# amzn/MXFusion

Measured on AMD Instinct MI355X. Metric: ELBO-steps/sec + RBF Gram GB/s, SVGP N=65k D=8 M=1024, 1->8 MI355X, higher is better.
Workload: dtype f32; 1 GPU; SVGPRegression RBF-ARD N=65536 Q=8 M=1024, 32 MC samples (latent-input model), StochasticVariationalInference step = draw + ELBO + reverse mode + grad all-reduce + Adam; samples_per_gpu=32, parallelism=mc-samples sharded x1, 1 RCCL all-reduce of the flat gradient/step, core_precision=float64 (M x M factorisations), streaming float32

## Files before the change

### mxfusion_amd/csrc/gemm_bt.hip

```cpp
#include "common.h"
#include "internal.h"
#include "split_device.h"

namespace {

typedef short s16x4 __attribute__((ext_vector_type(4)));

struct BtArgs {
    const unsigned short* A; const unsigned short* Bt; float* C;
    int64_t M, N, K16;
    int64_t pA, pB, btR;
    float alpha;
    int c_blk;
    int64_t ldc;
    int64_t tm, tn, nwg;
    const float* ad0;
    const unsigned* maxbits;
    const unsigned* maxbits2;
    unsigned* maxout;
    unsigned* sync; int sync_n;
    int sync_every;
    const unsigned short* uw; const unsigned* uwmax; float* uout; float uscale;
};

__device__ __forceinline__ void bt_dma16(const void* sbase, unsigned voff, unsigned lds) {
    asm volatile("s_mov_b32 m0, %2\n\ts_nop 0\n\tglobal_load_lds_dwordx4 %0, %1" ::"v"(voff), "s"(sbase), "s"(lds) : "memory", "m0");
}

__device__ __forceinline__ float bt_dot8(u32x4 a, u32x4 b, float acc) {
    const f16x8 av = __builtin_bit_cast(f16x8, a), bv = __builtin_bit_cast(f16x8, b);
    acc = __builtin_amdgcn_fdot2(f16x2{av[0], av[1]}, f16x2{bv[0], bv[1]}, acc, false);
    acc = __builtin_amdgcn_fdot2(f16x2{av[2], av[3]}, f16x2{bv[2], bv[3]}, acc, false);
    acc = __builtin_amdgcn_fdot2(f16x2{av[4], av[5]}, f16x2{bv[4], bv[5]}, acc, false);
    acc = __builtin_amdgcn_fdot2(f16x2{av[6], av[7]}, f16x2{bv[6], bv[7]}, acc, false);
    return acc;
}

constexpr int BT_KMAX16 = 128;

template <bool WU>
__global__ __launch_bounds__(512, 2) void gemm_f16x2_bt_kernel(BtArgs g) {
    constexpr int NU = 512;
    __shared__ u32x4 sA[4][2][NU];
    __shared__ u32x4 sB[4][2][NU];
    __shared__ u32x4 sW[WU ? 2 * BT_KMAX16 * 2 : 1];
    __shared__ float sU[WU ? 512 : 1];
    const int tid = threadIdx.x, lane = tid & 63, wave = tid >> 6, wq = wave & 3, wh = wave >> 2;
    const int li = lane & 31, lk = lane >> 5;
    int patience = 2;
    float cmax = 0.f;
    if constexpr (WU) {
        if (g.uout) {
            const int nunits = (int)(g.K16 * 2);
            for (int i = tid; i < 2 * nunits; i += 512) {
                const int p = i / nunits, u = i % nunits;
                sW[p * (BT_KMAX16 * 2) + u] = *reinterpret_cast<const u32x4*>(g.uw + (int64_t)p * g.K16 * 16 + u * 8);
            }
        }
        __syncthreads();
    }
    float alpha = g.alpha;
    if (g.ad0) alpha *= g.ad0[0];
    if (g.maxbits) alpha /= scale_from_maxbits(g.maxbits[0]);
    if (g.maxbits2) alpha /= scale_from_maxbits(g.maxbits2[0]);

    const int drow = tid >> 1, dkh = (tid & 1) ^ ((drow >> 3) & 1);
    const int bc = tid >> 3, bs = tid & 7;
    const int b_nb = 4 * (bc >> 4) + 2 * ((bc >> 3) & 1) + (bc & 1);
    const int b_kl = 8 * ((bc >> 1) & 1) + 4 * ((bc >> 2) & 1) + (bs >> 1);
    const unsigned voff_b = (unsigned)((((int64_t)b_nb * g.btR + b_kl) * 16 + 8 * (bs & 1)) * 2);
    const unsigned voff_a = (unsigned)((drow * 16 + dkh * 8) * 2);
    const int ua0_ = lds_unit(128 * wh + li, lk);
#define ua_(x) (ua0_ + 64 * (x))
    const unsigned ldsA = __builtin_amdgcn_readfirstlane((unsigned)(size_t)(__attribute__((address_space(3))) void*)&sA[0][0][wave * 64]);
    const unsigned ldsB = __builtin_amdgcn_readfirstlane((unsigned)(size_t)(__attribute__((address_space(3))) void*)&sB[0][0][wave * 64]);
    const unsigned toff_blk = (unsigned)((((int64_t)(4 * wq) * g.M + 128 * wh + li) * 16 + 4 * lk) * 4);
    const int rb_h = (wq * 2048 + (lane >> 4) * 128 + ((lane & 15) >> 2) * 32 + (lane & 3) * 8) / 2;

    const int nk = (int)g.K16;
    const unsigned nwg = (unsigned)g.nwg, tmu = (unsigned)g.tm;
    const int nit = (int)((nwg - blockIdx.x + gridDim.x - 1) / gridDim.x);
    const int nsteps = nit * nk;
    const unsigned q8 = nwg / 8, r8 = nwg % 8;
    auto item_of = [&](int i) -> unsigned { return xcd_run_item(blockIdx.x + (unsigned)i * gridDim.x, q8, r8); };
    int q_it = 0, q_kb = 0;
    unsigned q_slot = 0;
    const unsigned short* qa = nullptr;
    const unsigned short* qb = nullptr;
    auto q_enter = [&]() {
        const unsigned wid = item_of(q_it);
        const unsigned tn_ = wid / tmu, tm_ = wid - tn_ * tmu;
        qa = g.A + (int64_t)tm_ * 256 * 16;
        qb = g.Bt + ((int64_t)tn_ * 16) * g.btR * 16;
    };
    auto q_issue = [&]() {
        bt_dma16(qa + (int64_t)q_kb * g.M * 16, voff_a, ldsA + q_slot * 16384);
        bt_dma16(qa + g.pA + (int64_t)q_kb * g.M * 16, voff_a, ldsA + q_slot * 16384 + 8192);
        bt_dma16(qb + (int64_t)q_kb * 256, voff_b, ldsB + q_slot * 16384);
        bt_dma16(qb + g.pB + (int64_t)q_kb * 256, voff_b, ldsB + q_slot * 16384 + 8192);
        q_slot = (q_slot + 1) & 3;
        if (++q_kb == nk) { q_kb = 0; ++q_it; if (q_it < nit) q_enter(); }
    };
#define BT_WAIT(NSTR) do { asm volatile("s_waitcnt vmcnt(" NSTR ")" ::: "memory"); __builtin_amdgcn_s_barrier(); asm volatile("" ::: "memory"); } while (0)
#define HF(v) __builtin_bit_cast(f16x8, v)
#define BT_TR(ptr) __builtin_bit_cast(u32x2, __builtin_amdgcn_ds_read_tr16_b64_v4i16((__attribute__((address_space(3))) s16x4*)(ptr)))
    f32x16 c[4][2];
    float ua0 = 0.f, ua1 = 0.f;
    int c_kb = 0, c_it = 0;
    int64_t m0 = 0, n0 = 0;
    unsigned c_slot = 0;
    bool uitem = false;
    u32x4 fb0[2][2], fa0[2];
    u32x4 dga[6];
#define BT_READ_B(FB, SLOTV)                                                                                                        \
    do {                                                                                                                            \
        _Pragma("unroll") for (int p = 0; p < 2; ++p) {                                                                             \
            const unsigned short* sb_ = reinterpret_cast<const unsigned short*>(&sB[SLOTV][p][0]) + rb_h;                           \
            _Pragma("unroll") for (int y = 0; y < 2; ++y) {                                                                         \
                const u32x2 v0_ = BT_TR(sb_ + (2 * y) * 256), v1_ = BT_TR(sb_ + (2 * y + 1) * 256);                                 \
                FB[y][p] = u32x4{v0_[0], v0_[1], v1_[0], v1_[1]};                                                                   \
            }                                                                                                                       \
        }                                                                                                                           \
    } while (0)
#define BT_READ_A0(FA, SLOTV) do { FA[0] = sA[SLOTV][0][ua_(0)]; FA[1] = sA[SLOTV][1][ua_(0)]; } while (0)
#define BT_MM(x, AH, AL, FB)                                                                                                        \
    do {                                                                                                                            \
        _Pragma("unroll") for (int y = 0; y < 2; ++y) {                                                                             \
            c[x][y] = __builtin_amdgcn_mfma_f32_32x32x16_f16(HF(FB[y][0]), HF(AL), c[x][y], 0, 0, 0);                   \
            c[x][y] = __builtin_amdgcn_mfma_f32_32x32x16_f16(HF(FB[y][1]), HF(AH), c[x][y], 0, 0, 0);                   \
            c[x][y] = __builtin_amdgcn_mfma_f32_32x32x16_f16(HF(FB[y][0]), HF(AH), c[x][y], 0, 0, 0);                   \
        }                                                                                                                           \
    } while (0)
#define BT_STEP(FB, FA)                                                                                                   \
    do {                                                                                                                            \
        if (c_kb == 0) {                                                                        \
            const unsigned wid = item_of(c_it);                                                                                     \
            const unsigned tile_n = wid / tmu, tile_m = wid - tile_n * tmu;                                                         \
            m0 = (int64_t)tile_m * 256; n0 = (int64_t)tile_n * 256;                                                                 \
            uitem = WU && g.uout != nullptr && ((tile_n + (tile_n >> 3) + (tile_n >> 6)) % tmu) == tile_m;                          \
            if (g.sync && (c_it % g.sync_every) == 0) wg_rendezvous(g.sync + wid / g.sync_n, (unsigned)g.sync_n, patience);         \
            _Pragma("unroll") for (int x = 0; x < 4; ++x)                                                                           \
                _Pragma("unroll") for (int y = 0; y < 2; ++y)                                                                       \
                    _Pragma("unroll") for (int r = 0; r < 16; ++r) c[x][y][r] = 0.f;                                                \
            ua0 = 0.f; ua1 = 0.f;                                                                                                   \
        }                                                                                                                           \
        const bool more = s_ + 3 < nsteps;                                                                                          \
        if (more) q_issue();                                                      \
        asm volatile("" ::: "memory");                                             \
        const unsigned nslot = (c_slot + 1) & 3;                                                                                    \
        BT_READ_B(FB, c_slot);                                                                                                      \
        BT_READ_A0(FA, c_slot);                                                                                                     \
        if constexpr (WU) {                                                                                                         \
            if (uitem && (((int)c_kb & 1) == wh)) {                              \
                const u32x4 wh_ = sW[2 * (int)c_kb + lk], wl_ = sW[BT_KMAX16 * 2 + 2 * (int)c_kb + lk];                             \
                ua0 = bt_dot8(FB[0][1], wh_, ua0); ua0 = bt_dot8(FB[0][0], wl_, ua0); ua0 = bt_dot8(FB[0][0], wh_, ua0);            \
                ua1 = bt_dot8(FB[1][1], wh_, ua1); ua1 = bt_dot8(FB[1][0], wl_, ua1); ua1 = bt_dot8(FB[1][0], wh_, ua1);            \
            }                                                                                                                       \
        }                                                                                                                           \
         \
        dga[0] = sA[c_slot][0][ua_(1)]; dga[1] = sA[c_slot][1][ua_(1)]; dga[2] = sA[c_slot][0][ua_(2)]; dga[3] = sA[c_slot][1][ua_(2)];      \
        u32x4 a1h = dga[0], a1l = dga[1];                                                                                           \
        u32x4 a2h = dga[2], a2l = dga[3];                                                                                           \
        BT_MM(0, FA[0], FA[1], FB);                                                                                                 \
        __builtin_amdgcn_sched_barrier(0);               \
        dga[4] = sA[c_slot][0][ua_(3)]; dga[5] = sA[c_slot][1][ua_(3)];                                                             \
        u32x4 a3h = dga[4], a3l = dga[5];                                                                                           \
        BT_MM(1, a1h, a1l, FB);                                                                                                     \
        __builtin_amdgcn_sched_barrier(0);                                                                                          \
        BT_MM(2, a2h, a2l, FB);                                                                                                     \
        __builtin_amdgcn_sched_barrier(0);                                                                                          \
        BT_MM(3, a3h, a3l, FB);                                                                                                     \
        __builtin_amdgcn_sched_barrier(0);                                                                                          \
        if (more) BT_WAIT("8"); else if (s_ + 2 < nsteps) BT_WAIT("4"); else BT_WAIT("0");                        \
        c_slot = nslot;                                                                                                             \
        if (++c_kb == nk) { c_kb = 0; ++c_it; finish_item(); }                                                                      \
        ++s_;                                                                                                                       \
    } while (0)
    auto finish_item = [&]() {
        if constexpr (WU) {
            if (uitem) {
                ua0 += __shfl_xor(ua0, 32, 64);
                ua1 += __shfl_xor(ua1, 32, 64);
                if (lane < 32) { sU[256 * wh + 64 * wq + li] = ua0; sU[256 * wh + 64 * wq + 32 + li] = ua1; }
                __syncthreads();
                if (tid < 256) {
                    float sc = g.uscale * (g.ad0 ? g.ad0[0] : 1.f) / scale_from_maxbits(g.uwmax[0]);
                    if (g.maxbits2) sc /= scale_from_maxbits(g.maxbits2[0]);
                    g.uout[n0 + tid] = (sU[tid] + sU[256 + tid]) * sc;
                }
            }
        }
        if (g.c_blk) {
            char* const cb = reinterpret_cast<char*>(g.C) + ((n0 >> 4) * g.M + m0) * 64;
#pragma unroll
            for (int x = 0; x < 4; ++x)
#pragma unroll
                for (int y = 0; y < 2; ++y)
#pragma unroll
                    for (int q = 0; q < 4; ++q) {
                        char* const sb = cb + ((int64_t)(2 * y + (q >> 1)) * g.M + 32 * x) * 64 + 32 * (q & 1);
                        const f32x4 v = {alpha * c[x][y][4 * q], alpha * c[x][y][4 * q + 1], alpha * c[x][y][4 * q + 2], alpha * c[x][y][4 * q + 3]};
                        *reinterpret_cast<f32x4*>(sb + toff_blk) = v;
                        if (g.maxout) cmax = fmaxf(fmaxf(cmax, fmaxf(fabsf(v[0]), fabsf(v[1]))), fmaxf(fabsf(v[2]), fabsf(v[3])));
                    }
        } else {
#pragma unroll
            for (int x = 0; x < 4; ++x) {
                const int64_t row = m0 + 128 * wh + 32 * x + li;
#pragma unroll
                for (int y = 0; y < 2; ++y)
#pragma unroll
                    for (int q = 0; q < 4; ++q) {
                        const int64_t col = n0 + 64 * wq + 32 * y + 8 * q + 4 * lk;
                        float* p = g.C + row * g.ldc + col;
                        const f32x4 v = {alpha * c[x][y][4 * q], alpha * c[x][y][4 * q + 1], alpha * c[x][y][4 * q + 2], alpha * c[x][y][4 * q + 3]};
                        *reinterpret_cast<f32x4*>(p) = v;
                        if (g.maxout) cmax = fmaxf(fmaxf(cmax, fmaxf(fabsf(v[0]), fabsf(v[1]))), fmaxf(fabsf(v[2]), fabsf(v[3])));
                    }
            }
        }
    };
    if (nsteps > 0) {
        q_enter();
        q_issue();
        q_issue();
        q_issue();
        BT_WAIT("8");
    }
    int s_ = 0;
    while (s_ < nsteps) BT_STEP(fb0, fa0);
#undef ua_
#undef BT_STEP
#undef BT_MM
#undef BT_READ_A0
#undef BT_READ_B
#undef BT_TR
#undef HF
#undef BT_WAIT
    if (g.maxout) {
#pragma unroll
        for (int o = 32; o > 0; o >>= 1) cmax = fmaxf(cmax, __shfl_xor(cmax, o, 64));
        if (lane == 0 && __builtin_bit_cast(unsigned, cmax) > *(volatile unsigned*)g.maxout) atomicMax(g.maxout, __builtin_bit_cast(unsigned, cmax));
    }
}

__global__ __launch_bounds__(256) void bt_wsplit_kernel(int64_t K, int64_t Kp, const float* __restrict__ w, unsigned short* __restrict__ planes,
                                                        unsigned* __restrict__ maxword) {
    __shared__ unsigned wm[4];
    unsigned m = 0;
    for (int64_t i = threadIdx.x; i < K; i += 256) { const unsigned b = __builtin_bit_cast(unsigned, w[i]) & 0x7fffffffu; m = b > m ? b : m; }
    for (int o = 32; o > 0; o >>= 1) { const unsigned t = (unsigned)__shfl_xor((int)m, o); m = t > m ? t : m; }
    if ((threadIdx.x & 63) == 0) wm[threadIdx.x >> 6] = m;
    __syncthreads();
    for (int i = 0; i < 4; ++i) m = wm[i] > m ? wm[i] : m;
    if (threadIdx.x == 0) maxword[0] = m;
    const float sc = scale_from_maxbits(m);
    for (int64_t i = threadIdx.x; i < Kp; i += 256) {
        const float x = i < K ? w[i] * sc : 0.f;
        const _Float16 fh = (_Float16)x;
        const _Float16 fl = (_Float16)(x - (float)fh);
        planes[i] = __builtin_bit_cast(unsigned short, fh);
        planes[Kp + i] = __builtin_bit_cast(unsigned short, fl);
    }
}

}

bool mxf_gemm_bt_ok(int64_t M, int64_t N, int64_t K) { return M > 0 && N > 0 && K >= 48 && (M % 256) == 0 && (N % 256) == 0 && (K % 16) == 0; }

namespace {

struct BtPlan { BtArgs g; unsigned grid; unsigned ncounters; const float* w; unsigned short* wplanes; unsigned* wmax; };

int bt_plan(mxf_ctx* h, int64_t M, int64_t N, int64_t K, const MxfSplitScale& sc, const MxfPlanes& A, const MxfPlanes& Bt, int64_t btR,
            const MxfSplitOut& o, const MxfBtURow& u, const MxfSplitSched& sched, BtPlan& p) {
    if (o.planes || o.planes_t || o.avec || o.a_lower || o.lower_only || o.beta != 0.0 || sc.pow0 < 0 || sc.pow0 > 1)
        MXF_FAIL(h, -2, "mxf_gemm_bt: the output is C or blocked C of a full product with beta == 0, and ad0 enters once");
    if (o.blocked && M * 16 * 64 >= (1ll << 31)) MXF_FAIL(h, -3, "mxf_gemm_bt: too many rows for the blocked output");
    if (btR * 16 * 32 >= (1ll << 31)) MXF_FAIL(h, -3, "mxf_gemm_bt: the K-major operand has too many rows");
    if (!mxf_gemm_bt_ok(M, N, K) || btR < K) MXF_FAIL(h, -2, "mxf_gemm_bt: needs M %% 256 == 0, N %% 256 == 0, K %% 16 == 0, K >= 48");
    if (o.blocked && o.ldc != N) MXF_FAIL(h, -2, "mxf_gemm_bt: the blocked output layout needs ldc == N");
    if ((o.ldc % 4) != 0 || (((uintptr_t)o.C) % 16) != 0) MXF_FAIL(h, -2, "mxf_gemm_bt: C must be 16-byte aligned with ldc %% 4 == 0");
    if (u.U && (!u.w || !u.wscratch || K / 16 > BT_KMAX16)) MXF_FAIL(h, -2, "mxf_gemm_bt: the U row needs w, scratch and K <= %d", BT_KMAX16 * 16);
    BtArgs& g = p.g;
    memset(&g, 0, sizeof(g));
    g.A = A.p; g.pA = A.stride; g.maxbits = A.maxbits; g.Bt = Bt.p; g.pB = Bt.stride; g.maxbits2 = Bt.maxbits; g.btR = btR;
    g.M = M; g.N = N; g.K16 = K / 16; g.tm = M / 256; g.tn = N / 256; g.nwg = g.tm * g.tn;
    g.alpha = (float)sc.alpha; g.ad0 = sc.pow0 ? sc.ad0 : nullptr;
    g.C = o.C; g.ldc = o.ldc; g.c_blk = o.blocked; g.maxout = o.maxout;
    p.w = u.w; p.wplanes = nullptr; p.wmax = nullptr;
    if (u.U) {
        p.wplanes = (unsigned short*)u.wscratch; p.wmax = (unsigned*)(p.wplanes + 2 * K);
        g.uw = p.wplanes; g.uwmax = p.wmax; g.uout = u.U; g.uscale = (float)u.uscale;
    }
    int64_t grid = (int64_t)(256 - (sched.reserve_cus > 0 ? sched.reserve_cus : 0)) / 8 * 8;
    if (grid < 8) grid = 8;
    if (g.nwg <= grid) grid = g.nwg;
    p.grid = (unsigned)grid;
    static const int sync_env = (int)MXF_KNOB("MXF_BT_SYNC", 4);
    p.ncounters = 0;
    if (sync_env && strip_rendezvous_ok(g.tm, g.nwg, grid)) {
        p.ncounters = (unsigned)(g.nwg / g.tm);
        g.sync_n = (int)g.tm; g.sync_every = sync_env > 0 ? sync_env : 1;
    }
    return 0;
}

int bt_launch(mxf_ctx* h, hipStream_t st, BtPlan& p) {
    BtArgs& g = p.g;
    if (g.uout) hipLaunchKernelGGL(bt_wsplit_kernel, dim3(1), dim3(256), 0, st, g.K16 * 16, g.K16 * 16, p.w, p.wplanes, p.wmax);
    if (p.ncounters) g.sync = mxf_gsync(h, p.ncounters);
    if (g.uout) hipLaunchKernelGGL((gemm_f16x2_bt_kernel<true>), dim3(p.grid), dim3(512), 0, st, g);
    else hipLaunchKernelGGL((gemm_f16x2_bt_kernel<false>), dim3(p.grid), dim3(512), 0, st, g);
    MXF_LAUNCH_CHECK(h);
    return 0;
}

}

int mxf_gemm_bt_internal(mxf_ctx* h, hipStream_t st, int64_t M, int64_t N, int64_t K, MxfSplitScale scale, MxfPlanes A, MxfPlanes Bt, int64_t btR,
                         MxfSplitOut out, MxfBtURow u, MxfSplitSched sched) {
    BtPlan p;
    const int rc = bt_plan(h, M, N, K, scale, A, Bt, btR, out, u, sched, p);
    return rc ? rc : bt_launch(h, st, p);
}

extern "C" int mxf_gemm_f16x2_planes_kmajor(mxf_handle h, int64_t M, int64_t N, int64_t K, double alpha, const void* A_planes, const void* A_maxword,
                                            const void* Bt_planes, const void* Bt_maxword, void* C, int blocked, const void* w, void* U, void* stream) {
    if (!h) return -1;
    if (!A_planes || !Bt_planes || !A_maxword || !Bt_maxword || !C || ((w == nullptr) != (U == nullptr))) MXF_FAIL(h, -2, "mxf_gemm_f16x2_planes_kmajor: bad argument");
    if (!mxf_gemm_bt_ok(M, N, K)) MXF_FAIL(h, -3, "mxf_gemm_f16x2_planes_kmajor: needs M %% 256 == 0, N %% 256 == 0, K %% 16 == 0, K >= 48");
    void* ws = nullptr;
    if (U) {
        ws = mxf_ws(h, mxf_align((2 * (size_t)K + 8) * 2));
        if (!ws) MXF_FAIL(h, -4, "mxf_gemm_f16x2_planes_kmajor: cannot allocate scratch");
    }
    return mxf_gemm_bt_internal(h, (hipStream_t)stream, M, N, K, {.alpha = alpha},
                                {(const unsigned short*)A_planes, (int64_t)mxf_split_plane_elems(M, K), (const unsigned*)A_maxword},
                                {(const unsigned short*)Bt_planes, (int64_t)mxf_split_plane_elems(K, N), (const unsigned*)Bt_maxword}, K,
                                {.C = (float*)C, .ldc = N, .blocked = blocked ? 1 : 0}, {.w = (const float*)w, .U = (float*)U, .wscratch = ws});
}
```

Before: 43.54 ELBO-steps/sec.

## Switch BT GEMM to 16x16x32 MFMA with K-pair double-buffered stages

Replaces the 32x32x16 MFMA tiling with 16x16x32 MFMA. Each pipeline stage now loads two K16 blocks into a 2-slot double buffer instead of one block into a 4-slot ring. The A and B LDS layouts, the per-lane index math and the epilogue mappings are reworked to match, and the item loop is restructured around an odd-K tail that masks the upper half-lanes. The goal is fewer waits and barriers per unit of K work and better MFMA issue density. In exchange, register pressure rises (8x4 accumulators plus 8 fragments), prefetch depth drops, and the LDS reads for the next stage are interleaved with a mid-step barrier.

After: 44.92 ELBO-steps/sec, median of 6. +3.2%, better.

```diff
diff --git a/mxfusion_amd/csrc/gemm_bt.hip b/mxfusion_amd/csrc/gemm_bt.hip
--- a/mxfusion_amd/csrc/gemm_bt.hip
+++ b/mxfusion_amd/csrc/gemm_bt.hip
@@ -41,20 +41,20 @@
 template <bool WU>
 __global__ __launch_bounds__(512, 2) void gemm_f16x2_bt_kernel(BtArgs g) {
     constexpr int NU = 512;
-    __shared__ u32x4 sA[4][2][NU];
-    __shared__ u32x4 sB[4][2][NU];
+    __shared__ u32x4 sA[2][2][2][NU];
+    __shared__ u32x4 sB[2][2][2][NU];
     __shared__ u32x4 sW[WU ? 2 * BT_KMAX16 * 2 : 1];
     __shared__ float sU[WU ? 512 : 1];
     const int tid = threadIdx.x, lane = tid & 63, wave = tid >> 6, wq = wave & 3, wh = wave >> 2;
-    const int li = lane & 31, lk = lane >> 5;
+    const int lj = lane & 15, lg = lane >> 4;
     int patience = 2;
     float cmax = 0.f;
     if constexpr (WU) {
         if (g.uout) {
-            const int nunits = (int)(g.K16 * 2);
-            for (int i = tid; i < 2 * nunits; i += 512) {
-                const int p = i / nunits, u = i % nunits;
-                sW[p * (BT_KMAX16 * 2) + u] = *reinterpret_cast<const u32x4*>(g.uw + (int64_t)p * g.K16 * 16 + u * 8);
+            const int nunits = (int)(g.K16 * 2), npad = (nunits + 3) & ~3;
+            for (int i = tid; i < 2 * npad; i += 512) {
+                const int p = i / npad, u = i % npad;
+                sW[p * (BT_KMAX16 * 2) + u] = u < nunits ? *reinterpret_cast<const u32x4*>(g.uw + (int64_t)p * g.K16 * 16 + u * 8) : u32x4{0u, 0u, 0u, 0u};
             }
         }
         __syncthreads();
@@ -64,26 +64,24 @@
     if (g.maxbits) alpha /= scale_from_maxbits(g.maxbits[0]);
     if (g.maxbits2) alpha /= scale_from_maxbits(g.maxbits2[0]);
 
-    const int drow = tid >> 1, dkh = (tid & 1) ^ ((drow >> 3) & 1);
     const int bc = tid >> 3, bs = tid & 7;
-    const int b_nb = 4 * (bc >> 4) + 2 * ((bc >> 3) & 1) + (bc & 1);
-    const int b_kl = 8 * ((bc >> 1) & 1) + 4 * ((bc >> 2) & 1) + (bs >> 1);
+    const int b_nb = bc >> 2;
+    const int b_kl = 8 * (bc & 1) + 4 * ((bc >> 1) & 1) + (bs >> 1);
     const unsigned voff_b = (unsigned)((((int64_t)b_nb * g.btR + b_kl) * 16 + 8 * (bs & 1)) * 2);
-    const unsigned voff_a = (unsigned)((drow * 16 + dkh * 8) * 2);
-    const int ua0_ = lds_unit(128 * wh + li, lk);
-#define ua_(x) (ua0_ + 64 * (x))
-    const unsigned ldsA = __builtin_amdgcn_readfirstlane((unsigned)(size_t)(__attribute__((address_space(3))) void*)&sA[0][0][wave * 64]);
-    const unsigned ldsB = __builtin_amdgcn_readfirstlane((unsigned)(size_t)(__attribute__((address_space(3))) void*)&sB[0][0][wave * 64]);
-    const unsigned toff_blk = (unsigned)((((int64_t)(4 * wq) * g.M + 128 * wh + li) * 16 + 4 * lk) * 4);
-    const int rb_h = (wq * 2048 + (lane >> 4) * 128 + ((lane & 15) >> 2) * 32 + (lane & 3) * 8) / 2;
-
-    const int nk = (int)g.K16;
+    const unsigned voff_a = (unsigned)(tid * 16);
+    const int ua0_ = (128 * wh + lj) * 2 + (lg & 1) + (lg >> 1) * (2 * NU);
+    const unsigned ldsA = __builtin_amdgcn_readfirstlane((unsigned)(size_t)(__attribute__((address_space(3))) void*)&sA[0][0][0][wave * 64]);
+    const unsigned ldsB = __builtin_amdgcn_readfirstlane((unsigned)(size_t)(__attribute__((address_space(3))) void*)&sB[0][0][0][wave * 64]);
+    const unsigned toff_blk = (unsigned)((((int64_t)(4 * wq) * g.M + 128 * wh + lj) * 16 + 4 * lg) * 4);
+    const int rb_h = (wq * 2048 + (lg >> 1) * 16384 + (lg & 1) * 128 + (lj >> 2) * 32 + (lj & 3) * 8) / 2;
+
+    const int nk = (int)g.K16, np = (nk + 1) / 2;
     const unsigned nwg = (unsigned)g.nwg, tmu = (unsigned)g.tm;
     const int nit = (int)((nwg - blockIdx.x + gridDim.x - 1) / gridDim.x);
-    const int nsteps = nit * nk;
+    const int nsteps = nit * np;
     const unsigned q8 = nwg / 8, r8 = nwg % 8;
     auto item_of = [&](int i) -> unsigned { return xcd_run_item(blockIdx.x + (unsigned)i * gridDim.x, q8, r8); };
-    int q_it = 0, q_kb = 0;
+    int q_it = 0, q_p = 0;
     unsigned q_slot = 0;
     const unsigned short* qa = nullptr;
     const unsigned short* qb = nullptr;
@@ -94,94 +92,93 @@
         qb = g.Bt + ((int64_t)tn_ * 16) * g.btR * 16;
     };
     auto q_issue = [&]() {
-        bt_dma16(qa + (int64_t)q_kb * g.M * 16, voff_a, ldsA + q_slot * 16384);
-        bt_dma16(qa + g.pA + (int64_t)q_kb * g.M * 16, voff_a, ldsA + q_slot * 16384 + 8192);
-        bt_dma16(qb + (int64_t)q_kb * 256, voff_b, ldsB + q_slot * 16384);
-        bt_dma16(qb + g.pB + (int64_t)q_kb * 256, voff_b, ldsB + q_slot * 16384 + 8192);
-        q_slot = (q_slot + 1) & 3;
-        if (++q_kb == nk) { q_kb = 0; ++q_it; if (q_it < nit) q_enter(); }
+        const int kb0 = 2 * q_p, kb1 = kb0 + 1 < nk ? kb0 + 1 : kb0;
+        const unsigned la = ldsA + q_slot * 32768, lb = ldsB + q_slot * 32768;
+        bt_dma16(qa + (int64_t)kb0 * g.M * 16, voff_a, la);
+        bt_dma16(qa + g.pA + (int64_t)kb0 * g.M * 16, voff_a, la + 8192);
+        bt_dma16(qb + (int64_t)kb0 * 256, voff_b, lb);
+        bt_dma16(qb + g.pB + (int64_t)kb0 * 256, voff_b, lb + 8192);
+        bt_dma16(qa + (int64_t)kb1 * g.M * 16, voff_a, la + 16384);
+        bt_dma16(qa + g.pA + (int64_t)kb1 * g.M * 16, voff_a, la + 16384 + 8192);
+        bt_dma16(qb + (int64_t)kb1 * 256, voff_b, lb + 16384);
+        bt_dma16(qb + g.pB + (int64_t)kb1 * 256, voff_b, lb + 16384 + 8192);
+        q_slot ^= 1;
+        if (++q_p == np) { q_p = 0; ++q_it; if (q_it < nit) q_enter(); }
     };
 #define BT_WAIT(NSTR) do { asm volatile("s_waitcnt vmcnt(" NSTR ")" ::: "memory"); __builtin_amdgcn_s_barrier(); asm volatile("" ::: "memory"); } while (0)
 #define HF(v) __builtin_bit_cast(f16x8, v)
 #define BT_TR(ptr) __builtin_bit_cast(u32x2, __builtin_amdgcn_ds_read_tr16_b64_v4i16((__attribute__((address_space(3))) s16x4*)(ptr)))
-    f32x16 c[4][2];
-    float ua0 = 0.f, ua1 = 0.f;
-    int c_kb = 0, c_it = 0;
+    f32x4 c[8][4];
+    float ua[4] = {0.f, 0.f, 0.f, 0.f};
     int64_t m0 = 0, n0 = 0;
     unsigned c_slot = 0;
     bool uitem = false;
-    u32x4 fb0[2][2], fa0[2];
-    u32x4 dga[6];
-#define BT_READ_B(FB, SLOTV)                                                                                                        \
+    u32x4 fb[4][2];
+#define BT_A(x, p) sa_[(p) * NU + ua0_ + 32 * (x)]
+#define BT_MM(x, AH, AL)                                                                                                           \
     do {                                                                                                                            \
+        _Pragma("unroll") for (int t = 0; t < 4; ++t) {                                                                             \
+            c[x][t] = __builtin_amdgcn_mfma_f32_16x16x32_f16(HF(fb[t][0]), HF(AL), c[x][t], 0, 0, 0);                   \
+            c[x][t] = __builtin_amdgcn_mfma_f32_16x16x32_f16(HF(fb[t][1]), HF(AH), c[x][t], 0, 0, 0);                   \
+            c[x][t] = __builtin_amdgcn_mfma_f32_16x16x32_f16(HF(fb[t][0]), HF(AH), c[x][t], 0, 0, 0);                   \
+        }                                                                                                                           \
+        __builtin_amdgcn_sched_barrier(0);               \
+    } while (0)
+#define BT_STEP(TAIL)                                                                                                              \
+    do {                                                                                                                            \
+        const u32x4* const sa_ = &sA[c_slot][0][0][0];                                                                              \
         _Pragma("unroll") for (int p = 0; p < 2; ++p) {                                                                             \
-            const unsigned short* sb_ = reinterpret_cast<const unsigned short*>(&sB[SLOTV][p][0]) + rb_h;                           \
-            _Pragma("unroll") for (int y = 0; y < 2; ++y) {                                                                         \
-                const u32x2 v0_ = BT_TR(sb_ + (2 * y) * 256), v1_ = BT_TR(sb_ + (2 * y + 1) * 256);                                 \
-                FB[y][p] = u32x4{v0_[0], v0_[1], v1_[0], v1_[1]};                                                                   \
+            const unsigned short* sb_ = reinterpret_cast<const unsigned short*>(&sB[c_slot][0][p][0]) + rb_h;                       \
+            _Pragma("unroll") for (int t = 0; t < 4; ++t) {                                                                         \
+                const u32x2 v0_ = BT_TR(sb_ + t * 256), v1_ = BT_TR(sb_ + t * 256 + 128);                                           \
+                fb[t][p] = u32x4{v0_[0], v0_[1], v1_[0], v1_[1]};                                                                   \
+                if (TAIL) fb[t][p] &= kmask;            \
             }                                                                                                                       \
         }                                                                                                                           \
-    } while (0)
-#define BT_READ_A0(FA, SLOTV) do { FA[0] = sA[SLOTV][0][ua_(0)]; FA[1] = sA[SLOTV][1][ua_(0)]; } while (0)
-#define BT_MM(x, AH, AL, FB)                                                                                                        \
-    do {                                                                                                                            \
-        _Pragma("unroll") for (int y = 0; y < 2; ++y) {                                                                             \
-            c[x][y] = __builtin_amdgcn_mfma_f32_32x32x16_f16(HF(FB[y][0]), HF(AL), c[x][y], 0, 0, 0);                   \
-            c[x][y] = __builtin_amdgcn_mfma_f32_32x32x16_f16(HF(FB[y][1]), HF(AH), c[x][y], 0, 0, 0);                   \
-            c[x][y] = __builtin_amdgcn_mfma_f32_32x32x16_f16(HF(FB[y][0]), HF(AH), c[x][y], 0, 0, 0);                   \
-        }                                                                                                                           \
-    } while (0)
-#define BT_STEP(FB, FA)                                                                                                   \
-    do {                                                                                                                            \
-        if (c_kb == 0) {                                                                        \
-            const unsigned wid = item_of(c_it);                                                                                     \
-            const unsigned tile_n = wid / tmu, tile_m = wid - tile_n * tmu;                                                         \
-            m0 = (int64_t)tile_m * 256; n0 = (int64_t)tile_n * 256;                                                                 \
-            uitem = WU && g.uout != nullptr && ((tile_n + (tile_n >> 3) + (tile_n >> 6)) % tmu) == tile_m;                          \
-            if (g.sync && (c_it % g.sync_every) == 0) wg_rendezvous(g.sync + wid / g.sync_n, (unsigned)g.sync_n, patience);         \
-            _Pragma("unroll") for (int x = 0; x < 4; ++x)                                                                           \
-                _Pragma("unroll") for (int y = 0; y < 2; ++y)                                                                       \
-                    _Pragma("unroll") for (int r = 0; r < 16; ++r) c[x][y][r] = 0.f;                                                \
-            ua0 = 0.f; ua1 = 0.f;                                                                                                   \
-        }                                                                                                                           \
-        const bool more = s_ + 3 < nsteps;                                                                                          \
-        if (more) q_issue();                                                      \
-        asm volatile("" ::: "memory");                                             \
-        const unsigned nslot = (c_slot + 1) & 3;                                                                                    \
-        BT_READ_B(FB, c_slot);                                                                                                      \
-        BT_READ_A0(FA, c_slot);                                                                                                     \
+        u32x4 a0h = BT_A(0, 0), a0l = BT_A(0, 1), a1h = BT_A(1, 0), a1l = BT_A(1, 1);                                           \
         if constexpr (WU) {                                                                                                         \
-            if (uitem && (((int)c_kb & 1) == wh)) {                              \
-                const u32x4 wh_ = sW[2 * (int)c_kb + lk], wl_ = sW[BT_KMAX16 * 2 + 2 * (int)c_kb + lk];                             \
-                ua0 = bt_dot8(FB[0][1], wh_, ua0); ua0 = bt_dot8(FB[0][0], wl_, ua0); ua0 = bt_dot8(FB[0][0], wh_, ua0);            \
-                ua1 = bt_dot8(FB[1][1], wh_, ua1); ua1 = bt_dot8(FB[1][0], wl_, ua1); ua1 = bt_dot8(FB[1][0], wh_, ua1);            \
+            if (uitem && ((c_p & 1) == wh)) {                                 \
+                const u32x4 wh_ = sW[4 * c_p + lg], wl_ = sW[BT_KMAX16 * 2 + 4 * c_p + lg];                                         \
+                _Pragma("unroll") for (int t = 0; t < 4; ++t) {                                                                     \
+                    ua[t] = bt_dot8(fb[t][1], wh_, ua[t]); ua[t] = bt_dot8(fb[t][0], wl_, ua[t]); ua[t] = bt_dot8(fb[t][0], wh_, ua[t]); \
+                }                                                                                                                   \
             }                                                                                                                       \
         }                                                                                                                           \
-         \
-        dga[0] = sA[c_slot][0][ua_(1)]; dga[1] = sA[c_slot][1][ua_(1)]; dga[2] = sA[c_slot][0][ua_(2)]; dga[3] = sA[c_slot][1][ua_(2)];      \
-        u32x4 a1h = dga[0], a1l = dga[1];                                                                                           \
-        u32x4 a2h = dga[2], a2l = dga[3];                                                                                           \
-        BT_MM(0, FA[0], FA[1], FB);                                                                                                 \
-        __builtin_amdgcn_sched_barrier(0);               \
-        dga[4] = sA[c_slot][0][ua_(3)]; dga[5] = sA[c_slot][1][ua_(3)];                                                             \
-        u32x4 a3h = dga[4], a3l = dga[5];                                                                                           \
-        BT_MM(1, a1h, a1l, FB);                                                                                                     \
-        __builtin_amdgcn_sched_barrier(0);                                                                                          \
-        BT_MM(2, a2h, a2l, FB);                                                                                                     \
-        __builtin_amdgcn_sched_barrier(0);                                                                                          \
-        BT_MM(3, a3h, a3l, FB);                                                                                                     \
-        __builtin_amdgcn_sched_barrier(0);                                                                                          \
-        if (more) BT_WAIT("8"); else if (s_ + 2 < nsteps) BT_WAIT("4"); else BT_WAIT("0");                        \
-        c_slot = nslot;                                                                                                             \
-        if (++c_kb == nk) { c_kb = 0; ++c_it; finish_item(); }                                                                      \
-        ++s_;                                                                                                                       \
+                                                               \
+        u32x4 a2h = BT_A(2, 0), a2l = BT_A(2, 1);                                                                                 \
+        BT_MM(0, a0h, a0l);                                                                                                        \
+        u32x4 a3h = BT_A(3, 0), a3l = BT_A(3, 1);                                                                                 \
+        BT_MM(1, a1h, a1l);                                                                                                        \
+        u32x4 a4h = BT_A(4, 0), a4l = BT_A(4, 1);                                                                                 \
+        BT_MM(2, a2h, a2l);                                                                                                        \
+        u32x4 a5h = BT_A(5, 0), a5l = BT_A(5, 1);                                                                                 \
+        BT_MM(3, a3h, a3l);                                                                                                        \
+        u32x4 a6h = BT_A(6, 0), a6l = BT_A(6, 1);                                                                                 \
+        BT_MM(4, a4h, a4l);                                                                                                        \
+        u32x4 a7h = BT_A(7, 0), a7l = BT_A(7, 1);                                                                                 \
+        BT_MM(5, a5h, a5l);                                                                                                        \
+                     \
+        asm volatile("s_waitcnt lgkmcnt(0)" ::: "memory");                                                                          \
+        __builtin_amdgcn_s_barrier();                                                                                               \
+        asm volatile("" ::: "memory");                                                                                              \
+        const bool more = s_ + 2 < nsteps;                                                                                          \
+        if (more) q_issue();                                                                                                        \
+        asm volatile("" ::: "memory");                                                                                              \
+        BT_MM(6, a6h, a6l);                                                                                                        \
+        BT_MM(7, a7h, a7l);                                                                                                        \
+            \
+        if (more) BT_WAIT("8"); else BT_WAIT("0");                                                                                  \
+        c_slot ^= 1; ++c_p; ++s_;                                                                                                   \
     } while (0)
     auto finish_item = [&]() {
         if constexpr (WU) {
             if (uitem) {
-                ua0 += __shfl_xor(ua0, 32, 64);
-                ua1 += __shfl_xor(ua1, 32, 64);
-                if (lane < 32) { sU[256 * wh + 64 * wq + li] = ua0; sU[256 * wh + 64 * wq + 32 + li] = ua1; }
+#pragma unroll
+                for (int t = 0; t < 4; ++t) {
+                    ua[t] += __shfl_xor(ua[t], 16, 64);
+                    ua[t] += __shfl_xor(ua[t], 32, 64);
+                    if (lane < 16) sU[256 * wh + 64 * wq + 16 * t + lj] = ua[t];
+                }
                 __syncthreads();
                 if (tid < 256) {
                     float sc = g.uscale * (g.ad0 ? g.ad0[0] : 1.f) / scale_from_maxbits(g.uwmax[0]);
@@ -193,47 +190,58 @@
         if (g.c_blk) {
             char* const cb = reinterpret_cast<char*>(g.C) + ((n0 >> 4) * g.M + m0) * 64;
 #pragma unroll
-            for (int x = 0; x < 4; ++x)
-#pragma unroll
-                for (int y = 0; y < 2; ++y)
-#pragma unroll
-                    for (int q = 0; q < 4; ++q) {
-                        char* const sb = cb + ((int64_t)(2 * y + (q >> 1)) * g.M + 32 * x) * 64 + 32 * (q & 1);
-                        const f32x4 v = {alpha * c[x][y][4 * q], alpha * c[x][y][4 * q + 1], alpha * c[x][y][4 * q + 2], alpha * c[x][y][4 * q + 3]};
-                        *reinterpret_cast<f32x4*>(sb + toff_blk) = v;
-                        if (g.maxout) cmax = fmaxf(fmaxf(cmax, fmaxf(fabsf(v[0]), fabsf(v[1]))), fmaxf(fabsf(v[2]), fabsf(v[3])));
-                    }
+            for (int x = 0; x < 8; ++x)
+#pragma unroll
+                for (int t = 0; t < 4; ++t) {
+                    char* const sb = cb + ((int64_t)t * g.M + 16 * x) * 64;
+                    const f32x4 v = {alpha * c[x][t][0], alpha * c[x][t][1], alpha * c[x][t][2], alpha * c[x][t][3]};
+                    *reinterpret_cast<f32x4*>(sb + toff_blk) = v;
+                    if (g.maxout) cmax = fmaxf(fmaxf(cmax, fmaxf(fabsf(v[0]), fabsf(v[1]))), fmaxf(fabsf(v[2]), fabsf(v[3])));
+                }
         } else {
 #pragma unroll
-            for (int x = 0; x < 4; ++x) {
-                const int64_t row = m0 + 128 * wh + 32 * x + li;
-#pragma unroll
-                for (int y = 0; y < 2; ++y)
-#pragma unroll
-                    for (int q = 0; q < 4; ++q) {
-                        const int64_t col = n0 + 64 * wq + 32 * y + 8 * q + 4 * lk;
-                        float* p = g.C + row * g.ldc + col;
-                        const f32x4 v = {alpha * c[x][y][4 * q], alpha * c[x][y][4 * q + 1], alpha * c[x][y][4 * q + 2], alpha * c[x][y][4 * q + 3]};
-                        *reinterpret_cast<f32x4*>(p) = v;
-                        if (g.maxout) cmax = fmaxf(fmaxf(cmax, fmaxf(fabsf(v[0]), fabsf(v[1]))), fmaxf(fabsf(v[2]), fabsf(v[3])));
-                    }
+            for (int x = 0; x < 8; ++x) {
+                const int64_t row = m0 + 128 * wh + 16 * x + lj;
+#pragma unroll
+                for (int t = 0; t < 4; ++t) {
+                    const int64_t col = n0 + 64 * wq + 16 * t + 4 * lg;
+                    float* p = g.C + row * g.ldc + col;
+                    const f32x4 v = {alpha * c[x][t][0], alpha * c[x][t][1], alpha * c[x][t][2], alpha * c[x][t][3]};
+                    *reinterpret_cast<f32x4*>(p) = v;
+                    if (g.maxout) cmax = fmaxf(fmaxf(cmax, fmaxf(fabsf(v[0]), fabsf(v[1]))), fmaxf(fabsf(v[2]), fabsf(v[3])));
+                }
             }
         }
     };
+    const unsigned kmask = lane < 32 ? ~0u : 0u;
     if (nsteps > 0) {
         q_enter();
         q_issue();
-        q_issue();
-        q_issue();
-        BT_WAIT("8");
+        if (nsteps > 1) { q_issue(); BT_WAIT("8"); } else BT_WAIT("0");
     }
     int s_ = 0;
-    while (s_ < nsteps) BT_STEP(fb0, fa0);
-#undef ua_
+    for (int c_it = 0; c_it < nit; ++c_it) {
+        {
+            const unsigned wid = item_of(c_it);
+            const unsigned tile_n = wid / tmu, tile_m = wid - tile_n * tmu;
+            m0 = (int64_t)tile_m * 256; n0 = (int64_t)tile_n * 256;
+            uitem = WU && g.uout != nullptr && ((tile_n + (tile_n >> 3) + (tile_n >> 6)) % tmu) == tile_m;
+            if (g.sync && (c_it % g.sync_every) == 0) wg_rendezvous(g.sync + wid / g.sync_n, (unsigned)g.sync_n, patience);
+#pragma unroll
+            for (int x = 0; x < 8; ++x)
+#pragma unroll
+                for (int t = 0; t < 4; ++t) c[x][t] = f32x4{0.f, 0.f, 0.f, 0.f};
+#pragma unroll
+            for (int t = 0; t < 4; ++t) ua[t] = 0.f;
+        }
+        int c_p = 0;
+        while (c_p < nk / 2) BT_STEP(false);
+        if (nk & 1) BT_STEP(true);
+        finish_item();
+    }
 #undef BT_STEP
 #undef BT_MM
-#undef BT_READ_A0
-#undef BT_READ_B
+#undef BT_A
 #undef BT_TR
 #undef HF
 #undef BT_WAIT
```
